# uber-research/UPSNet

Measured on NVIDIA H100. Metric: panoptic images/sec at 1024x2048, higher is better.
Workload: dtype bf16x3

## Files before the change

upsnet_b200/csrc/dcn_win.cu:

```cuda
#include <cuda.h>
#include <cuda_bf16.h>

#include "common.cuh"
#include "tc_ptx.cuh"
#include "tc_params.cuh"

namespace ups {

constexpr int DW_BM = 128;
constexpr int DW_WW = 32, DW_WH = 20;
constexpr int DW_PLANE = DW_WW * DW_WH * 32;
constexpr int DW_WIN_BYTES = 2 * DW_PLANE;
constexpr int DW_WIN_BUFS = 2;
constexpr int DW_KHW = 9;
constexpr int DW_GROUPS = 2;
constexpr int DW_EPI_PITCH = 36;
constexpr uint32_t DW_EPI_BYTES = DW_BM * DW_EPI_PITCH * 4;

constexpr uint32_t DW_OFF_BARS = 0;
constexpr uint32_t DW_OFF_STATS = 192;
constexpr uint32_t DW_OFF_ORG = 256;
constexpr uint32_t DW_OFF_TW = 512;
constexpr uint32_t DW_OFF_TP = DW_OFF_TW + DW_KHW * DW_BM * 16;
constexpr uint32_t DW_OFF_STAGES = DW_OFF_TP + DW_KHW * DW_BM * 4;
static_assert(DW_OFF_STAGES % 1024 == 0, "stage buffers need 1024-byte alignment (SWIZZLE_128B)");

template <int BN> struct DwCfg {
  static constexpr int NCW = BN == 128 ? 2 : 1;
  static constexpr int FRAGS = 2 / NCW;
  static constexpr int BK = BN == 128 ? 32 : 64;
  static constexpr int SPK = BK / 16;
  static constexpr int ROWB = BK * 2;
  static constexpr int CONSUMERS = 128 * NCW;
  static constexpr int WARP_TMAB = CONSUMERS / 32, WARP_TMAW = WARP_TMAB + 1, WARP_PROD0 = WARP_TMAB + 4;
  static constexpr int GROUP = 4 * (SPK / 2) * 32;
  static constexpr int PRODUCERS = GROUP * DW_GROUPS;
  static constexpr int THREADS = WARP_PROD0 * 32 + PRODUCERS;
  static constexpr int WARPGROUPS = THREADS / 128;
  static constexpr int REGS_LAUNCH = 16384 / (32 * ((THREADS / 32 + 3) / 4)) / 8 * 8;
  static constexpr int REGS_TMA = 32, REGS_CONSUMER = 128;
  static_assert(NCW * REGS_CONSUMER + REGS_TMA + (PRODUCERS / 128) * REGS_LAUNCH <= WARPGROUPS * REGS_LAUNCH,
                "setmaxnreg budgets exceed the CTA's register allocation");
  static constexpr int TABLE_IT = (DW_KHW * DW_BM + PRODUCERS - 1) / PRODUCERS;
  static constexpr uint32_t A_BYTES = 2 * DW_BM * ROWB;
  static constexpr uint32_t B_BYTES = BN * ROWB;
  static constexpr uint32_t STAGE_BYTES = 2 * B_BYTES + A_BYTES;
  static_assert(STAGE_BYTES % 1024 == 0, "stages must keep the 1024-byte alignment of the swizzled tiles");
  static constexpr int STAGES = BN == 128 ? 3 : 2;
  static_assert(STAGES <= 3, "the barrier map holds three stages");
  static constexpr uint32_t OFF_WIN = DW_OFF_STAGES + STAGES * STAGE_BYTES;
  static constexpr uint32_t OFF_EPI = OFF_WIN + DW_WIN_BUFS * DW_WIN_BYTES;
  static constexpr uint32_t SMEM = OFF_EPI + DW_EPI_BYTES + 1024;
  static_assert(SMEM <= 227 * 1024, "shared memory exceeds 227 KB");
};
template <int ROWB> __device__ __forceinline__ uint32_t dw_chunk(uint32_t j, uint32_t r) {
  return ROWB == 128 ? (j ^ (r & 7u)) : (j ^ ((r >> 1) & 3u));
}

struct DwParams {
  const void* x;
  const float* offset;
  const float* mask;
  const float* bias;
  void* y;
  int N, H, W, Cin, Cout, Cout_pad, Ho, Wo, ph, pw, dh, dw, relu, BN, tile_w, tile_h;
};

template <int BN>
__global__ void __launch_bounds__(DwCfg<BN>::THREADS, 1)
dcn_win_kernel(const __grid_constant__ CUtensorMap tm_x, const __grid_constant__ CUtensorMap tm_w, const __grid_constant__ DwParams p) {
  using C = DwCfg<BN>;
  constexpr int DW_PRODUCERS = C::PRODUCERS, DW_CONSUMERS = C::CONSUMERS;
  constexpr int DW_WARP_TMAB = C::WARP_TMAB, DW_WARP_TMAW = C::WARP_TMAW, DW_WARP_PROD0 = C::WARP_PROD0;
  constexpr int DW_BK = C::BK, SPK = C::SPK, ROWB = C::ROWB;
  extern __shared__ __align__(1024) uint8_t smem_dyn[];
  const uint32_t raw = smem_u32(smem_dyn);
  const uint32_t base = (raw + 1023u) & ~1023u;
  uint8_t* sm = smem_dyn + (base - raw);

  const int tid = threadIdx.x, warp = tid >> 5, lane = tid & 31;
  const uint32_t b_bytes = C::B_BYTES;
  const uint32_t stage_bytes = C::STAGE_BYTES;
  constexpr uint32_t NST = C::STAGES, NWB = DW_WIN_BUFS;
  const uint32_t win_base = base + C::OFF_WIN;
  float* stf = reinterpret_cast<float*>(sm + C::OFF_EPI);
  const uint32_t bar_fa = base + DW_OFF_BARS;
  const uint32_t bar_fb = bar_fa + 24;
  const uint32_t bar_em = bar_fa + 48;
  const uint32_t bar_wf = bar_fa + 104;
  const uint32_t bar_we = bar_fa + 120;
  const uint32_t bar_og = bar_fa + 136;
  int* stats = reinterpret_cast<int*>(sm + DW_OFF_STATS);
  int4* org = reinterpret_cast<int4*>(sm + DW_OFF_ORG);
  float4* tw = reinterpret_cast<float4*>(sm + DW_OFF_TW);
  int* tp = reinterpret_cast<int*>(sm + DW_OFF_TP);

  const int HoWo = p.Ho * p.Wo;
  const int nsc = p.Cin / 16;
  const int num_kb = nsc * DW_KHW / SPK;
  const int n_tiles = p.Cout_pad / BN;
  const int TW = p.tile_w, TH = p.tile_h;
  const int tw_shift = TW == 16 ? 4 : 3;
  const int tiles_w = (p.Wo + TW - 1) / TW, tiles_h = (p.Ho + TH - 1) / TH;
  const long long num_tiles = (long long)p.N * tiles_w * tiles_h * n_tiles;

  if (warp == 0) {
    if (lane == 0) {
      for (int s = 0; s < C::STAGES; ++s) {
        mbar_init(bar_fa + 8 * s, C::GROUP / 32);
        mbar_init(bar_fb + 8 * s, 1);
        mbar_init(bar_em + 8 * s, DW_CONSUMERS / 32);
      }
      for (int s = 0; s < 2; ++s) {
        mbar_init(bar_wf + 8 * s, 1);
        mbar_init(bar_we + 8 * s, DW_PRODUCERS / 32);
        mbar_init(bar_og + 8 * s, 1);
      }
      fence_mbar_init();
      for (int i = 0; i < 2; ++i) {
        stats[i * 8 + 0] = 0x7fffffff; stats[i * 8 + 1] = 0x7fffffff;
        stats[i * 8 + 2] = -0x7fffffff; stats[i * 8 + 3] = -0x7fffffff;
        stats[i * 8 + 4] = 0; stats[i * 8 + 5] = 0; stats[i * 8 + 6] = 0; stats[i * 8 + 7] = 0;
      }
    }
    __syncwarp();
  }
  if (warp == DW_WARP_TMAB && lane == 0) prefetch_tmap(&tm_w);
  if (warp == DW_WARP_TMAW && lane == 0) prefetch_tmap(&tm_x);
  __syncthreads();

  if (warp >= DW_WARP_PROD0) {
    const int pt = tid - DW_WARP_PROD0 * 32;
    const int pw = warp - DW_WARP_PROD0;
    const int group = pw / (C::GROUP / 32);
    const int u = (pw >> 2) & (SPK / 2 - 1);
    const int quad = pw & 3;
    const int r = quad * 32 + lane;
    const __nv_bfloat16* xh = reinterpret_cast<const __nv_bfloat16*>(p.x);
    uint32_t g0 = 0, wf0 = 0;
    uint32_t wf_ready = 0;
    uint32_t tile_it = 0;
    for (long long tile = blockIdx.x; tile < num_tiles; tile += gridDim.x, ++tile_it) {
      const long long mt = tile / n_tiles;
      const int tx = (int)(mt % tiles_w), ty = (int)((mt / tiles_w) % tiles_h), n = (int)(mt / ((long long)tiles_w * tiles_h));
      const int par = (int)(tile_it & 1u);
      constexpr int TIT = C::TABLE_IT;
      float4 ewv[TIT];
      int ehl[TIT], ewl[TIT];
      bool evalid[TIT];
      int mnw = 0x7fffffff, mnh = 0x7fffffff, mxw = -0x7fffffff, mxh = -0x7fffffff, sw_ = 0, sh_ = 0, cnt = 0;
#pragma unroll
      for (int it = 0; it < TIT; ++it) {
        const int e = pt + it * DW_PRODUCERS;
        ewv[it] = make_float4(0.f, 0.f, 0.f, 0.f);
        ehl[it] = 0; ewl[it] = 0; evalid[it] = false;
        if (e < DW_KHW * DW_BM) {
          const int tap = e >> 7, rr = e & 127;
          const int ry = rr >> tw_shift;
          const int wo = tx * TW + (rr & (TW - 1)), ho = ty * TH + ry;
          if (ry < TH && wo < p.Wo && ho < p.Ho) {
            const int pp = ho * p.Wo + wo;
            const int ki = tap / 3, kj = tap - ki * 3;
            const float* offp = p.offset + ((size_t)n * 2 * DW_KHW + 2 * tap) * HoWo + pp;
            const float oh = __ldg(offp), ow = __ldg(offp + HoWo);
            const float h = (float)(ho - p.ph + ki * p.dh) + oh;
            const float w = (float)(wo - p.pw + kj * p.dw) + ow;
            if (h > -1.f && w > -1.f && h < (float)p.H && w < (float)p.W) {
              const int hl = (int)floorf(h), wl = (int)floorf(w), hh = hl + 1, wh = wl + 1;
              const float lh = h - hl, lw = w - wl, ch = 1.f - lh, cw = 1.f - lw;
              const bool t_ok = hl >= 0, b_ok = hh <= p.H - 1, l_ok = wl >= 0, r_ok = wh <= p.W - 1;
              float m = 1.f;
              if (p.mask) m = __ldg(p.mask + ((size_t)n * DW_KHW + tap) * HoWo + pp);
              ewv[it].x = (t_ok && l_ok) ? ch * cw * m : 0.f;
              ewv[it].y = (t_ok && r_ok) ? ch * lw * m : 0.f;
              ewv[it].z = (b_ok && l_ok) ? lh * cw * m : 0.f;
              ewv[it].w = (b_ok && r_ok) ? lh * lw * m : 0.f;
              ehl[it] = hl; ewl[it] = wl; evalid[it] = true;
              mnw = min(mnw, wl); mxw = max(mxw, wl + 1); mnh = min(mnh, hl); mxh = max(mxh, hl + 1);
              sw_ += wl; sh_ += hl; ++cnt;
            }
          }
        }
      }
      mnw = __reduce_min_sync(0xffffffffu, mnw); mnh = __reduce_min_sync(0xffffffffu, mnh);
      mxw = __reduce_max_sync(0xffffffffu, mxw); mxh = __reduce_max_sync(0xffffffffu, mxh);
      sw_ = __reduce_add_sync(0xffffffffu, sw_); sh_ = __reduce_add_sync(0xffffffffu, sh_);
      cnt = __reduce_add_sync(0xffffffffu, cnt);
      if (lane == 0 && cnt > 0) {
        int* st = stats + par * 8;
        atomicMin(st + 0, mnw); atomicMin(st + 1, mnh); atomicMax(st + 2, mxw); atomicMax(st + 3, mxh);
        atomicAdd(st + 4, sw_); atomicAdd(st + 5, sh_); atomicAdd(st + 6, cnt);
      }
      named_bar<1, DW_PRODUCERS>();
      int ox = 0, oy = 0;
      {
        const int* st = stats + par * 8;
        const int c = st[6];
        if (c > 0) {
          const int a = st[0], b = st[1], cc = st[2], d = st[3];
          ox = (cc - a + 1 <= DW_WW) ? a : (int)floorf((float)st[4] / (float)c + 1.0f) - DW_WW / 2;
          oy = (d - b + 1 <= DW_WH) ? b : (int)floorf((float)st[5] / (float)c + 1.0f) - DW_WH / 2;
        }
      }
#pragma unroll
      for (int it = 0; it < TIT; ++it) {
        const int e = pt + it * DW_PRODUCERS;
        if (e < DW_KHW * DW_BM) {
          int code = 0;
          if (evalid[it]) {
            const int dx = ewl[it] - ox, dy = ehl[it] - oy;
            if (dx >= 0 && dx + 1 < DW_WW && dy >= 0 && dy + 1 < DW_WH) code = (dy * DW_WW + dx) * 32;
            else code = (int)(0x80000000u | ((uint32_t)(ehl[it] + 1) << 15) | (uint32_t)(ewl[it] + 1));
          }
          tw[e] = ewv[it];
          tp[e] = code;
        }
      }
      if (pt == 0) {
        org[par] = make_int4(ox, oy, n, 0);
        int* so = stats + (par ^ 1) * 8;
        so[0] = 0x7fffffff; so[1] = 0x7fffffff; so[2] = -0x7fffffff; so[3] = -0x7fffffff; so[4] = 0; so[5] = 0; so[6] = 0;
        mbar_arrive(bar_og + 8 * par);
      }
      named_bar<1, DW_PRODUCERS>();
      const __nv_bfloat16* ximg = xh + (size_t)n * p.H * p.W * (size_t)(2 * p.Cin);

      int rel = 0;
      for (int kb = (int)((uint32_t)(group - (int)g0) & 1u); kb < num_kb; kb += DW_GROUPS) {
        const uint32_t g = g0 + (uint32_t)kb;
        const uint32_t s = g % NST, it = g / NST;
        mbar_wait(bar_em + 8 * s, (it & 1u) ^ 1u);
        const uint32_t a_row = base + DW_OFF_STAGES + s * stage_bytes + 2 * b_bytes + (uint32_t)r * (uint32_t)ROWB;
#pragma unroll 1
        for (int pass = 0; pass < 4; ++pass) {
          const int sl = 2 * u + (pass >> 1), half = pass & 1;
          const int q = kb * SPK + sl;
          const int sc = q / DW_KHW, tap = q - sc * DW_KHW;
          const uint32_t wf = wf0 + (uint32_t)sc;
          if (wf >= wf_ready) {
            mbar_wait(bar_wf + 8 * (wf % NWB), (wf / NWB) & 1u);
            wf_ready = wf + 1;
          }
          const uint32_t wbuf = win_base + (wf % NWB) * (uint32_t)DW_WIN_BYTES;
          const int code = tp[tap * DW_BM + r];
          const uint32_t a_off = dw_chunk<ROWB>((uint32_t)(sl * 2 + half), (uint32_t)r) << 4;
          const float4 wv = tw[tap * DW_BM + r];
          uint4 hc[4], lc[4];
          if (code >= 0) {
            const uint32_t cl = (uint32_t)code, cr = cl + 32u;
            const uint32_t al = wbuf + cl + ((((cl >> 7) & 1u) ^ (uint32_t)half) << 4);
            const uint32_t ar = wbuf + cr + ((((cr >> 7) & 1u) ^ (uint32_t)half) << 4);
            hc[0] = lds128(al); hc[1] = lds128(ar); hc[2] = lds128(al + DW_WW * 32); hc[3] = lds128(ar + DW_WW * 32);
            lc[0] = lds128(al + DW_PLANE); lc[1] = lds128(ar + DW_PLANE);
            lc[2] = lds128(al + DW_PLANE + DW_WW * 32); lc[3] = lds128(ar + DW_PLANE + DW_WW * 32);
          } else {
            const int hl = (int)(((uint32_t)code >> 15) & 0xffffu) - 1, wl = (int)((uint32_t)code & 0x7fffu) - 1;
            const int h0 = max(hl, 0), h1 = min(hl + 1, p.H - 1), w0 = max(wl, 0), w1 = min(wl + 1, p.W - 1);
            const size_t pc = (size_t)(2 * p.Cin);
            const int cg = sc * 16 + half * 8;
            const __nv_bfloat16* b00 = ximg + ((size_t)h0 * p.W + w0) * pc + cg;
            const __nv_bfloat16* b01 = ximg + ((size_t)h0 * p.W + w1) * pc + cg;
            const __nv_bfloat16* b10 = ximg + ((size_t)h1 * p.W + w0) * pc + cg;
            const __nv_bfloat16* b11 = ximg + ((size_t)h1 * p.W + w1) * pc + cg;
            hc[0] = __ldg(reinterpret_cast<const uint4*>(b00)); lc[0] = __ldg(reinterpret_cast<const uint4*>(b00 + p.Cin));
            hc[1] = __ldg(reinterpret_cast<const uint4*>(b01)); lc[1] = __ldg(reinterpret_cast<const uint4*>(b01 + p.Cin));
            hc[2] = __ldg(reinterpret_cast<const uint4*>(b10)); lc[2] = __ldg(reinterpret_cast<const uint4*>(b10 + p.Cin));
            hc[3] = __ldg(reinterpret_cast<const uint4*>(b11)); lc[3] = __ldg(reinterpret_cast<const uint4*>(b11 + p.Cin));
          }
          const float wf4[4] = {wv.x, wv.y, wv.z, wv.w};
          unsigned long long acc[4] = {0ull, 0ull, 0ull, 0ull};
          __nv_bfloat162 lacc[4];
#pragma unroll
          for (int i = 0; i < 4; ++i) {
            const uint32_t hw_[4] = {hc[i].x, hc[i].y, hc[i].z, hc[i].w};
            const uint32_t lw_[4] = {lc[i].x, lc[i].y, lc[i].z, lc[i].w};
            const __nv_bfloat162 wb = __float2bfloat162_rn(wf4[i]);
            unsigned long long wp;
            asm("mov.b64 %0, {%1, %1};" : "=l"(wp) : "r"(__float_as_uint(wf4[i])));
#pragma unroll
            for (int qq = 0; qq < 4; ++qq) {
              unsigned long long hp;
              asm("mov.b64 %0, {%1, %2};" : "=l"(hp) : "r"(hw_[qq] << 16), "r"(hw_[qq] & 0xffff0000u));
              acc[qq] = f32x2_fma(wp, hp, acc[qq]);
              const __nv_bfloat162 lv = *reinterpret_cast<const __nv_bfloat162*>(&lw_[qq]);
              lacc[qq] = i == 0 ? __hmul2(wb, lv) : __hfma2(wb, lv, lacc[qq]);
            }
          }
          uint32_t ohi[4], olo[4];
#pragma unroll
          for (int qq = 0; qq < 4; ++qq) {
            const uint32_t lw = *reinterpret_cast<const uint32_t*>(&lacc[qq]);
            unsigned long long lp;
            asm("mov.b64 %0, {%1, %2};" : "=l"(lp) : "r"(lw << 16), "r"(lw & 0xffff0000u));
            acc[qq] = f32x2_add(acc[qq], lp);
            uint32_t a0, a1;
            asm("mov.b64 {%0, %1}, %2;" : "=r"(a0), "=r"(a1) : "l"(acc[qq]));
            const float v0 = __uint_as_float(a0), v1 = __uint_as_float(a1);
            ohi[qq] = pack_bf16x2(v0, v1);
            olo[qq] = pack_bf16x2(v0 - __uint_as_float(ohi[qq] << 16), v1 - __uint_as_float(ohi[qq] & 0xffff0000u));
          }
          sts128(a_row + a_off, make_uint4(ohi[0], ohi[1], ohi[2], ohi[3]));
          sts128(a_row + DW_BM * ROWB + a_off, make_uint4(olo[0], olo[1], olo[2], olo[3]));
        }
        fence_proxy_async();
        __syncwarp();
        if (lane == 0) {
          mbar_arrive(bar_fa + 8 * s);
          while (rel < nsc && DW_KHW * (rel + 1) <= SPK * (kb + DW_GROUPS)) {
            mbar_arrive(bar_we + 8 * ((wf0 + (uint32_t)rel) % NWB));
            ++rel;
          }
        }
        rel = __shfl_sync(0xffffffffu, rel, 0);
      }
      if (lane == 0) {
        while (rel < nsc) { mbar_arrive(bar_we + 8 * ((wf0 + (uint32_t)rel) % NWB)); ++rel; }
      }
      __syncwarp();
      g0 += (uint32_t)num_kb;
      wf0 += (uint32_t)nsc;
    }
  } else if (warp >= DW_WARP_TMAB) {
    setmaxnreg_dec<C::REGS_TMA>();
    if (warp == DW_WARP_TMAW && lane == 0) {
      uint32_t wf = 0, ti = 0;
      for (long long tile = blockIdx.x; tile < num_tiles; tile += gridDim.x, ++ti) {
        const uint32_t par = ti & 1u;
        mbar_wait(bar_og + 8 * par, (ti >> 1) & 1u);
        const volatile int* ov = reinterpret_cast<const volatile int*>(&org[par]);
        const int4 o = make_int4(ov[0], ov[1], ov[2], 0);
        for (int f = 0; f < nsc; ++f, ++wf) {
          const uint32_t b = wf % NWB;
          mbar_wait(bar_we + 8 * b, ((wf / NWB) & 1u) ^ 1u);
          mbar_arrive_expect_tx(bar_wf + 8 * b, (uint32_t)DW_WIN_BYTES);
          const uint32_t dst = win_base + b * (uint32_t)DW_WIN_BYTES;
          tma_load_4d(dst, &tm_x, bar_wf + 8 * b, f * 16, o.x, o.y, o.z);
          tma_load_4d(dst + (uint32_t)DW_PLANE, &tm_x, bar_wf + 8 * b, p.Cin + f * 16, o.x, o.y, o.z);
        }
      }
    } else if (warp == DW_WARP_TMAB && lane == 0) {
      uint32_t g = 0;
      for (long long tile = blockIdx.x; tile < num_tiles; tile += gridDim.x) {
        const int n0 = (int)(tile % n_tiles) * BN;
        for (int kb = 0; kb < num_kb; ++kb, ++g) {
          const uint32_t s = g % NST, it = g / NST;
          mbar_wait(bar_em + 8 * s, (it & 1u) ^ 1u);
          const uint32_t stage = base + DW_OFF_STAGES + s * stage_bytes;
          mbar_arrive_expect_tx(bar_fb + 8 * s, 2 * b_bytes);
          tma_load_2d(stage, &tm_w, bar_fb + 8 * s, kb * DW_BK, n0);
          tma_load_2d(stage + b_bytes, &tm_w, bar_fb + 8 * s, kb * DW_BK, p.Cout_pad + n0);
        }
      }
    }
    __syncwarp();
  } else {
    setmaxnreg_inc<C::REGS_CONSUMER>();
    constexpr int FRAGS = C::FRAGS;
    const int wg = warp >> 2;
    const uint32_t dhi = ROWB == 128 ? wg_desc_hi(8 * ROWB) : wg_desc_hi_sw64(8 * ROWB);
    float d[FRAGS][BN / 2];
    constexpr uint32_t h16 = 64u * ROWB / 16u;
    __nv_bfloat16* yb = reinterpret_cast<__nv_bfloat16*>(p.y);
    uint32_t s = 0, ph = 0;
    for (long long tile = blockIdx.x; tile < num_tiles; tile += gridDim.x) {
      const long long mt = tile / n_tiles;
      const int n0 = (int)(tile % n_tiles) * BN;
      const int tx = (int)(mt % tiles_w), ty = (int)((mt / tiles_w) % tiles_h), n = (int)(mt / ((long long)tiles_w * tiles_h));
      int prev = -1;
      for (int kb = 0; kb < num_kb; ++kb) {
        mbar_wait(bar_fb + 8 * s, ph);
        mbar_wait(bar_fa + 8 * s, ph);
        const uint32_t st0 = base + DW_OFF_STAGES + s * stage_bytes;
        const uint32_t b_hi = wg_desc_lo(st0), b_lo = wg_desc_lo(st0 + b_bytes);
        const uint32_t a_hi = wg_desc_lo(st0 + 2 * b_bytes) + (uint32_t)(wg * FRAGS) * h16;
        const uint32_t a_lo = wg_desc_lo(st0 + 2 * b_bytes + DW_BM * ROWB) + (uint32_t)(wg * FRAGS) * h16;
        wgmma_fence();
#pragma unroll
        for (uint32_t k = 0; k < SPK; ++k) {
          const uint32_t acc = (kb | k) ? 1u : 0u;
          const uint64_t bh = wg_desc(b_hi + 2 * k, dhi), bl = wg_desc(b_lo + 2 * k, dhi);
#pragma unroll
          for (int f = 0; f < FRAGS; ++f) Wgmma<BN>::mma(d[f], wg_desc(a_lo + f * h16 + 2 * k, dhi), bh, acc);
#pragma unroll
          for (int f = 0; f < FRAGS; ++f) Wgmma<BN>::mma(d[f], wg_desc(a_hi + f * h16 + 2 * k, dhi), bl, 1u);
#pragma unroll
          for (int f = 0; f < FRAGS; ++f) Wgmma<BN>::mma(d[f], wg_desc(a_hi + f * h16 + 2 * k, dhi), bh, 1u);
        }
        wgmma_commit();
        wgmma_wait<1>();
#pragma unroll
        for (int f = 0; f < FRAGS; ++f) wgmma_fence_acc(d[f]);
        if (prev >= 0 && lane == 0) mbar_arrive(bar_em + 8 * prev);
        prev = (int)s;
        if (++s == NST) { s = 0; ph ^= 1u; }
      }
      wgmma_wait<0>();
#pragma unroll
      for (int f = 0; f < FRAGS; ++f) wgmma_fence_acc(d[f]);
      if (prev >= 0 && lane == 0) mbar_arrive(bar_em + 8 * prev);

      const int t = tid & 127;
      const int m = FRAGS == 2 ? t : 64 * wg + (t & 63);
      const int csub = FRAGS == 2 ? 0 : 16 * (t >> 6), cstep = FRAGS == 2 ? 16 : 32;
      const int ry = m >> tw_shift;
      const int wo = tx * TW + (m & (TW - 1)), ho = ty * TH + ry;
      const bool row_ok = ry < TH && wo < p.Wo && ho < p.Ho;
      __nv_bfloat16* yp = yb + (((size_t)n * p.Ho + ho) * p.Wo + wo) * (size_t)(2 * p.Cout);
      const uint32_t trow = smem_u32(stf + (size_t)m * DW_EPI_PITCH);
      for (int c32 = 0; c32 < BN; c32 += 32) {
        if (n0 + c32 >= p.Cout) break;
        named_bar(2 + wg, 128);
#pragma unroll
        for (int c = 0; c < BN; c += 32)
          if (c == c32) {
#pragma unroll
            for (int f = 0; f < FRAGS; ++f) acc_stage<BN, 32>(d[f], stf, DW_EPI_PITCH, 64 * (wg * FRAGS + f), c);
          }
        named_bar(2 + wg, 128);
        for (int cb = c32 + csub; cb < c32 + 32 && cb < BN; cb += cstep) {
          if (n0 + cb >= p.Cout) break;
          uint32_t rr[16];
          acc_ld16(trow + (uint32_t)(cb - c32) * 4u, rr);
          if (!row_ok) continue;
          const int co = n0 + cb;
          float o[16];
#pragma unroll
          for (int e = 0; e < 16; ++e) o[e] = __uint_as_float(rr[e]);
          if (p.bias) {
            if (co + 16 <= p.Cout) {
#pragma unroll
              for (int e4 = 0; e4 < 4; ++e4) {
                const float4 bv = __ldg(reinterpret_cast<const float4*>(p.bias + co) + e4);
                o[4 * e4] += bv.x; o[4 * e4 + 1] += bv.y; o[4 * e4 + 2] += bv.z; o[4 * e4 + 3] += bv.w;
              }
            } else {
#pragma unroll
              for (int e = 0; e < 16; ++e)
                if (co + e < p.Cout) o[e] += __ldg(p.bias + co + e);
            }
          }
          if (p.relu) {
#pragma unroll
            for (int e = 0; e < 16; ++e) o[e] = fmaxf(o[e], 0.f);
          }
          uint32_t hw[8], lw[8];
#pragma unroll
          for (int e = 0; e < 8; ++e) {
            hw[e] = pack_bf16x2(o[2 * e], o[2 * e + 1]);
            lw[e] = pack_bf16x2(o[2 * e] - __uint_as_float(hw[e] << 16), o[2 * e + 1] - __uint_as_float(hw[e] & 0xffff0000u));
          }
          uint4* dh_ = reinterpret_cast<uint4*>(yp + co);
          uint4* dl_ = reinterpret_cast<uint4*>(yp + p.Cout + co);
          dh_[0] = make_uint4(hw[0], hw[1], hw[2], hw[3]); dh_[1] = make_uint4(hw[4], hw[5], hw[6], hw[7]);
          dl_[0] = make_uint4(lw[0], lw[1], lw[2], lw[3]); dl_[1] = make_uint4(lw[4], lw[5], lw[6], lw[7]);
        }
      }
    }
  }
}

__global__ void dcn_win_pack_kernel(const float* __restrict__ w, int Cout, int Cin, int Cout_pad, int K,
                                    uint16_t* __restrict__ hi, uint16_t* __restrict__ lo) {
  const size_t total = (size_t)Cout_pad * K;
  for (size_t i = (size_t)blockIdx.x * blockDim.x + threadIdx.x; i < total; i += (size_t)gridDim.x * blockDim.x) {
    const int kk = (int)(i % (size_t)K), co = (int)(i / (size_t)K);
    const int sc = kk / (16 * DW_KHW), rem = kk - sc * 16 * DW_KHW, tap = rem >> 4, c = sc * 16 + (rem & 15);
    const float v = co < Cout ? w[((size_t)co * Cin + c) * DW_KHW + tap] : 0.f;
    const __nv_bfloat16 h = __float2bfloat16_rn(v);
    const __nv_bfloat16 l = __float2bfloat16_rn(v - __bfloat162float(h));
    hi[i] = *reinterpret_cast<const uint16_t*>(&h);
    lo[i] = *reinterpret_cast<const uint16_t*>(&l);
  }
}

static bool dw_supported(int Cin, int Cout, int kh, int kw) {
  return kh == 3 && kw == 3 && Cin % 64 == 0 && Cin >= 64 && Cout >= 1;
}

}

extern "C" int upsnet_dcn_packed_weight_bytes(int Cout, int Cin, int kh, int kw, size_t* bytes) {
  if (!bytes || Cout <= 0 || Cin <= 0) return UPSNET_E_BADARG;
  if (!ups::dw_supported(Cin, Cout, kh, kw)) return UPSNET_E_UNSUPPORTED;
  *bytes = (size_t)2 * ups::cout_pad(Cout) * (size_t)(9 * Cin) * sizeof(uint16_t);
  return 0;
}

extern "C" int upsnet_dcn_pack_weight(const float* weight, int Cout, int Cin, int kh, int kw, void* packed, void* stream) {
  if (!weight || !packed || Cout <= 0 || Cin <= 0) return UPSNET_E_BADARG;
  if (!ups::dw_supported(Cin, Cout, kh, kw)) return UPSNET_E_UNSUPPORTED;
  const int Cout_pad = ups::cout_pad(Cout), K = 9 * Cin;
  uint16_t* hi = reinterpret_cast<uint16_t*>(packed);
  uint16_t* lo = hi + (size_t)Cout_pad * K;
  const size_t total = (size_t)Cout_pad * K;
  int blocks = (int)((total + 255) / 256);
  if (blocks > ups::kNumSMs * 16) blocks = ups::kNumSMs * 16;
  ups::dcn_win_pack_kernel<<<blocks, 256, 0, (cudaStream_t)stream>>>(weight, Cout, Cin, Cout_pad, K, hi, lo);
  UPS_CHECK_LAUNCH();
  return 0;
}

static int g_dw_force_bn = 0;

extern "C" int upsnet_dcn_set_tile_n(int bn) {
  if (bn != 0 && bn != 32 && bn != 128) return UPSNET_E_BADARG;
  g_dw_force_bn = bn;
  return 0;
}

extern "C" int upsnet_dcn_pair_forward(const void* x_pair, const float* offset, const float* mask, const void* packed,
                                       const float* bias, void* y_pair, int N, int H, int W, int Cin, int Cout, int kh,
                                       int kw, int pad_h, int pad_w, int dil_h, int dil_w, int epi_flags, void* stream) {
  using namespace ups;
  if (!x_pair || !offset || !packed || !y_pair) return UPSNET_E_BADARG;
  if (N <= 0 || H <= 0 || W <= 0 || Cin <= 0 || Cout <= 0 || pad_h < 0 || pad_w < 0 || dil_h <= 0 || dil_w <= 0) return UPSNET_E_BADARG;
  if (!dw_supported(Cin, Cout, kh, kw)) return UPSNET_E_UNSUPPORTED;
  if ((Cout % 16) != 0) return UPSNET_E_UNSUPPORTED;
  if (H >= 32767 || W >= 32767) return UPSNET_E_UNSUPPORTED;
  if ((((uintptr_t)x_pair) & 15) || (((uintptr_t)packed) & 15) || (((uintptr_t)y_pair) & 15) || (bias && (((uintptr_t)bias) & 15)))
    return UPSNET_E_UNSUPPORTED;
  DwParams p{};
  p.x = x_pair; p.offset = offset; p.mask = mask; p.bias = bias; p.y = y_pair;
  p.N = N; p.H = H; p.W = W; p.Cin = Cin; p.Cout = Cout; p.Cout_pad = cout_pad(Cout);
  p.ph = pad_h; p.pw = pad_w; p.dh = dil_h; p.dw = dil_w;
  p.Ho = conv_out_size(H, pad_h, dil_h, 3, 1);
  p.Wo = conv_out_size(W, pad_w, dil_w, 3, 1);
  if (p.Ho <= 0 || p.Wo <= 0) return UPSNET_E_BADARG;
  p.relu = (epi_flags & UPSNET_EPI_RELU) ? 1 : 0;
  const int sms = num_sms();
  p.tile_w = 16; p.tile_h = 8;
  auto dtiles = [&]() { return (long long)p.N * ((p.Wo + p.tile_w - 1) / p.tile_w) * ((p.Ho + p.tile_h - 1) / p.tile_h) * (p.Cout_pad / p.BN); };
  p.BN = 128;
  const bool wide_ok = p.Cout_pad % 128 == 0;
  const bool wide = wide_ok && (g_dw_force_bn == 128 || (g_dw_force_bn == 0 && dtiles() >= sms / 4));
  if (!wide) p.BN = 32;
  if (!wide && dtiles() < sms / 2) { p.tile_w = 8; p.tile_h = 8; }
  if (!wide && dtiles() < sms / 2) { p.tile_h = 4; }
  const long long num_tiles = dtiles();
  if (num_tiles <= 0) return 0;
  const int bk = wide ? DwCfg<128>::BK : DwCfg<32>::BK;
  const size_t smem = wide ? DwCfg<128>::SMEM : DwCfg<32>::SMEM;
  EncodeTiledFn enc = tma_encoder();
  if (!enc) return UPSNET_E_UNSUPPORTED;
  CUtensorMap tm_x, tm_w;
  {
    const cuuint64_t dx[4] = {(cuuint64_t)(2 * Cin), (cuuint64_t)W, (cuuint64_t)H, (cuuint64_t)N};
    const cuuint64_t sx[3] = {(cuuint64_t)(2 * Cin) * 2, (cuuint64_t)W * (2 * Cin) * 2, (cuuint64_t)H * W * (2 * Cin) * 2};
    const cuuint32_t bx[4] = {16, DW_WW, DW_WH, 1};
    const cuuint32_t es[4] = {1, 1, 1, 1};
    if (enc(&tm_x, CU_TENSOR_MAP_DATA_TYPE_BFLOAT16, 4, const_cast<void*>(x_pair), dx, sx, bx, es, CU_TENSOR_MAP_INTERLEAVE_NONE,
            CU_TENSOR_MAP_SWIZZLE_32B, CU_TENSOR_MAP_L2_PROMOTION_L2_128B, CU_TENSOR_MAP_FLOAT_OOB_FILL_NONE) != CUDA_SUCCESS)
      return UPSNET_E_UNSUPPORTED;
    const cuuint64_t dwt[2] = {(cuuint64_t)(9 * Cin), (cuuint64_t)(2 * p.Cout_pad)};
    const cuuint64_t sw[1] = {(cuuint64_t)(9 * Cin) * 2};
    const cuuint32_t bw[2] = {(cuuint32_t)bk, (cuuint32_t)p.BN};
    if (enc(&tm_w, CU_TENSOR_MAP_DATA_TYPE_BFLOAT16, 2, const_cast<void*>(packed), dwt, sw, bw, es, CU_TENSOR_MAP_INTERLEAVE_NONE,
            bk == 64 ? CU_TENSOR_MAP_SWIZZLE_128B : CU_TENSOR_MAP_SWIZZLE_64B, CU_TENSOR_MAP_L2_PROMOTION_L2_256B,
            CU_TENSOR_MAP_FLOAT_OOB_FILL_NONE) != CUDA_SUCCESS)
      return UPSNET_E_UNSUPPORTED;
  }
  static PerDeviceOnce configured;
  if (configured.need()) {
    UPS_CUDA(cudaFuncSetAttribute(dcn_win_kernel<32>, cudaFuncAttributeMaxDynamicSharedMemorySize, 227 * 1024));
    UPS_CUDA(cudaFuncSetAttribute(dcn_win_kernel<128>, cudaFuncAttributeMaxDynamicSharedMemorySize, 227 * 1024));
  }
  dim3 grid((unsigned)(num_tiles < sms ? num_tiles : sms));
  if (wide)
    dcn_win_kernel<128><<<grid, DwCfg<128>::THREADS, smem, (cudaStream_t)stream>>>(tm_x, tm_w, p);
  else
    dcn_win_kernel<32><<<grid, DwCfg<32>::THREADS, smem, (cudaStream_t)stream>>>(tm_x, tm_w, p);
  UPS_CHECK_LAUNCH();
  return 0;
}
```

Measured before the change: 127.9.

## Software-pipeline DCN producer window loads across passes and k-blocks

Restructures the deformable-conv producer loop so the high-plane corner loads for the next pass (and the next k-block when its window is already resident) are issued before the low-plane bf16 accumulation of the current pass. The pass loop is fully unrolled and the slice lookup is factored into lambdas. This is meant to hide shared-memory load latency behind FMA work. It also packs the per-entry hl/wl/valid into a single int and replaces a divide by 3 with a multiply-shift, at the cost of more live registers and more complex carry logic.

```diff
diff --git a/upsnet_b200/csrc/dcn_win.cu b/upsnet_b200/csrc/dcn_win.cu
--- a/upsnet_b200/csrc/dcn_win.cu
+++ b/upsnet_b200/csrc/dcn_win.cu
@@ -146,21 +146,21 @@
       const int par = (int)(tile_it & 1u);
       constexpr int TIT = C::TABLE_IT;
       float4 ewv[TIT];
-      int ehl[TIT], ewl[TIT];
-      bool evalid[TIT];
+      int ehw[TIT];
+
       int mnw = 0x7fffffff, mnh = 0x7fffffff, mxw = -0x7fffffff, mxh = -0x7fffffff, sw_ = 0, sh_ = 0, cnt = 0;
 #pragma unroll
       for (int it = 0; it < TIT; ++it) {
         const int e = pt + it * DW_PRODUCERS;
         ewv[it] = make_float4(0.f, 0.f, 0.f, 0.f);
-        ehl[it] = 0; ewl[it] = 0; evalid[it] = false;
+        ehw[it] = -1;
         if (e < DW_KHW * DW_BM) {
           const int tap = e >> 7, rr = e & 127;
           const int ry = rr >> tw_shift;
           const int wo = tx * TW + (rr & (TW - 1)), ho = ty * TH + ry;
           if (ry < TH && wo < p.Wo && ho < p.Ho) {
             const int pp = ho * p.Wo + wo;
-            const int ki = tap / 3, kj = tap - ki * 3;
+            const int ki = (tap * 11) >> 5, kj = tap - ki * 3;
             const float* offp = p.offset + ((size_t)n * 2 * DW_KHW + 2 * tap) * HoWo + pp;
             const float oh = __ldg(offp), ow = __ldg(offp + HoWo);
             const float h = (float)(ho - p.ph + ki * p.dh) + oh;
@@ -175,7 +175,7 @@
               ewv[it].y = (t_ok && r_ok) ? ch * lw * m : 0.f;
               ewv[it].z = (b_ok && l_ok) ? lh * cw * m : 0.f;
               ewv[it].w = (b_ok && r_ok) ? lh * lw * m : 0.f;
-              ehl[it] = hl; ewl[it] = wl; evalid[it] = true;
+              ehw[it] = ((hl + 1) << 16) | (wl + 1);
               mnw = min(mnw, wl); mxw = max(mxw, wl + 1); mnh = min(mnh, hl); mxh = max(mxh, hl + 1);
               sw_ += wl; sh_ += hl; ++cnt;
             }
@@ -207,10 +207,11 @@
         const int e = pt + it * DW_PRODUCERS;
         if (e < DW_KHW * DW_BM) {
           int code = 0;
-          if (evalid[it]) {
-            const int dx = ewl[it] - ox, dy = ehl[it] - oy;
+          if (ehw[it] >= 0) {
+            const int hl = (ehw[it] >> 16) - 1, wl = (ehw[it] & 0xffff) - 1;
+            const int dx = wl - ox, dy = hl - oy;
             if (dx >= 0 && dx + 1 < DW_WW && dy >= 0 && dy + 1 < DW_WH) code = (dy * DW_WW + dx) * 32;
-            else code = (int)(0x80000000u | ((uint32_t)(ehl[it] + 1) << 15) | (uint32_t)(ewl[it] + 1));
+            else code = (int)(0x80000000u | ((uint32_t)(hl + 1) << 15) | (uint32_t)(wl + 1));
           }
           tw[e] = ewv[it];
           tp[e] = code;
@@ -225,56 +226,76 @@
       named_bar<1, DW_PRODUCERS>();
       const __nv_bfloat16* ximg = xh + (size_t)n * p.H * p.W * (size_t)(2 * p.Cin);
 
+      auto win_corners = [&](int code, int half, uint32_t wbuf, uint32_t plane, uint4 (&c)[4]) {
+        const uint32_t cl = (uint32_t)code, cr = cl + 32u;
+        const uint32_t al = wbuf + plane + cl + ((((cl >> 7) & 1u) ^ (uint32_t)half) << 4);
+        const uint32_t ar = wbuf + plane + cr + ((((cr >> 7) & 1u) ^ (uint32_t)half) << 4);
+        c[0] = lds128(al); c[1] = lds128(ar); c[2] = lds128(al + DW_WW * 32); c[3] = lds128(ar + DW_WW * 32);
+      };
+      auto global_corners = [&](int code, int half, int sc, uint4 (&hc_)[4], uint4 (&lc_)[4]) {
+        const int hl = (int)(((uint32_t)code >> 15) & 0xffffu) - 1, wl = (int)((uint32_t)code & 0x7fffu) - 1;
+        const int h0 = max(hl, 0), h1 = min(hl + 1, p.H - 1), w0 = max(wl, 0), w1 = min(wl + 1, p.W - 1);
+        const size_t pc = (size_t)(2 * p.Cin);
+        const int cg = sc * 16 + half * 8;
+        const __nv_bfloat16* b00 = ximg + ((size_t)h0 * p.W + w0) * pc + cg;
+        const __nv_bfloat16* b01 = ximg + ((size_t)h0 * p.W + w1) * pc + cg;
+        const __nv_bfloat16* b10 = ximg + ((size_t)h1 * p.W + w0) * pc + cg;
+        const __nv_bfloat16* b11 = ximg + ((size_t)h1 * p.W + w1) * pc + cg;
+        hc_[0] = __ldg(reinterpret_cast<const uint4*>(b00)); lc_[0] = __ldg(reinterpret_cast<const uint4*>(b00 + p.Cin));
+        hc_[1] = __ldg(reinterpret_cast<const uint4*>(b01)); lc_[1] = __ldg(reinterpret_cast<const uint4*>(b01 + p.Cin));
+        hc_[2] = __ldg(reinterpret_cast<const uint4*>(b10)); lc_[2] = __ldg(reinterpret_cast<const uint4*>(b10 + p.Cin));
+        hc_[3] = __ldg(reinterpret_cast<const uint4*>(b11)); lc_[3] = __ldg(reinterpret_cast<const uint4*>(b11 + p.Cin));
+      };
+      auto slice = [&](int kb_, int sl_, int& sc_, int& tap_, int& code_, uint32_t& wbuf_) {
+        const int q = kb_ * SPK + sl_;
+        sc_ = q / DW_KHW;
+        tap_ = q - sc_ * DW_KHW;
+        code_ = tp[tap_ * DW_BM + r];
+        const uint32_t wf = wf0 + (uint32_t)sc_;
+        if (wf >= wf_ready) {
+          mbar_wait(bar_wf + 8 * (wf % NWB), (wf / NWB) & 1u);
+          wf_ready = wf + 1;
+        }
+        wbuf_ = win_base + (wf % NWB) * (uint32_t)DW_WIN_BYTES;
+      };
+
       int rel = 0;
-      for (int kb = (int)((uint32_t)(group - (int)g0) & 1u); kb < num_kb; kb += DW_GROUPS) {
+      const int kb0 = (int)((uint32_t)(group - (int)g0) & 1u);
+      int sc = 0, tap = 0, code = 0;
+      float4 wv = make_float4(0.f, 0.f, 0.f, 0.f);
+      uint32_t wbuf = 0;
+      uint4 hc[4];
+      bool carried = false;
+      for (int kb = kb0; kb < num_kb; kb += DW_GROUPS) {
+        if (!carried) {
+          slice(kb, 2 * u, sc, tap, code, wbuf);
+          wv = tw[tap * DW_BM + r];
+          if (code >= 0) win_corners(code, 0, wbuf, 0u, hc);
+        }
         const uint32_t g = g0 + (uint32_t)kb;
         const uint32_t s = g % NST, it = g / NST;
         mbar_wait(bar_em + 8 * s, (it & 1u) ^ 1u);
         const uint32_t a_row = base + DW_OFF_STAGES + s * stage_bytes + 2 * b_bytes + (uint32_t)r * (uint32_t)ROWB;
-#pragma unroll 1
+#pragma unroll
         for (int pass = 0; pass < 4; ++pass) {
           const int sl = 2 * u + (pass >> 1), half = pass & 1;
-          const int q = kb * SPK + sl;
-          const int sc = q / DW_KHW, tap = q - sc * DW_KHW;
-          const uint32_t wf = wf0 + (uint32_t)sc;
-          if (wf >= wf_ready) {
-            mbar_wait(bar_wf + 8 * (wf % NWB), (wf / NWB) & 1u);
-            wf_ready = wf + 1;
-          }
-          const uint32_t wbuf = win_base + (wf % NWB) * (uint32_t)DW_WIN_BYTES;
-          const int code = tp[tap * DW_BM + r];
-          const uint32_t a_off = dw_chunk<ROWB>((uint32_t)(sl * 2 + half), (uint32_t)r) << 4;
-          const float4 wv = tw[tap * DW_BM + r];
-          uint4 hc[4], lc[4];
-          if (code >= 0) {
-            const uint32_t cl = (uint32_t)code, cr = cl + 32u;
-            const uint32_t al = wbuf + cl + ((((cl >> 7) & 1u) ^ (uint32_t)half) << 4);
-            const uint32_t ar = wbuf + cr + ((((cr >> 7) & 1u) ^ (uint32_t)half) << 4);
-            hc[0] = lds128(al); hc[1] = lds128(ar); hc[2] = lds128(al + DW_WW * 32); hc[3] = lds128(ar + DW_WW * 32);
-            lc[0] = lds128(al + DW_PLANE); lc[1] = lds128(ar + DW_PLANE);
-            lc[2] = lds128(al + DW_PLANE + DW_WW * 32); lc[3] = lds128(ar + DW_PLANE + DW_WW * 32);
-          } else {
-            const int hl = (int)(((uint32_t)code >> 15) & 0xffffu) - 1, wl = (int)((uint32_t)code & 0x7fffu) - 1;
-            const int h0 = max(hl, 0), h1 = min(hl + 1, p.H - 1), w0 = max(wl, 0), w1 = min(wl + 1, p.W - 1);
-            const size_t pc = (size_t)(2 * p.Cin);
-            const int cg = sc * 16 + half * 8;
-            const __nv_bfloat16* b00 = ximg + ((size_t)h0 * p.W + w0) * pc + cg;
-            const __nv_bfloat16* b01 = ximg + ((size_t)h0 * p.W + w1) * pc + cg;
-            const __nv_bfloat16* b10 = ximg + ((size_t)h1 * p.W + w0) * pc + cg;
-            const __nv_bfloat16* b11 = ximg + ((size_t)h1 * p.W + w1) * pc + cg;
-            hc[0] = __ldg(reinterpret_cast<const uint4*>(b00)); lc[0] = __ldg(reinterpret_cast<const uint4*>(b00 + p.Cin));
-            hc[1] = __ldg(reinterpret_cast<const uint4*>(b01)); lc[1] = __ldg(reinterpret_cast<const uint4*>(b01 + p.Cin));
-            hc[2] = __ldg(reinterpret_cast<const uint4*>(b10)); lc[2] = __ldg(reinterpret_cast<const uint4*>(b10 + p.Cin));
-            hc[3] = __ldg(reinterpret_cast<const uint4*>(b11)); lc[3] = __ldg(reinterpret_cast<const uint4*>(b11 + p.Cin));
-          }
+          uint4 lc[4];
+          if (code >= 0) win_corners(code, half, wbuf, (uint32_t)DW_PLANE, lc);
+          else global_corners(code, half, sc, hc, lc);
+          int sc1 = sc, tap1 = tap, code1 = code;
+          uint32_t wbuf1 = wbuf;
+          if (pass == 3) {
+            const int f1 = ((kb + DW_GROUPS) * SPK + 2 * u) / DW_KHW;
+            carried = kb + DW_GROUPS < num_kb && DW_KHW * (f1 - 1) <= SPK * kb;
+          }
+          const bool more = pass < 3 || carried;
+          if (pass == 1) slice(kb, sl + 1, sc1, tap1, code1, wbuf1);
+          else if (pass == 3 && more) slice(kb + DW_GROUPS, 2 * u, sc1, tap1, code1, wbuf1);
           const float wf4[4] = {wv.x, wv.y, wv.z, wv.w};
           unsigned long long acc[4] = {0ull, 0ull, 0ull, 0ull};
-          __nv_bfloat162 lacc[4];
 #pragma unroll
           for (int i = 0; i < 4; ++i) {
             const uint32_t hw_[4] = {hc[i].x, hc[i].y, hc[i].z, hc[i].w};
-            const uint32_t lw_[4] = {lc[i].x, lc[i].y, lc[i].z, lc[i].w};
-            const __nv_bfloat162 wb = __float2bfloat162_rn(wf4[i]);
             unsigned long long wp;
             asm("mov.b64 %0, {%1, %1};" : "=l"(wp) : "r"(__float_as_uint(wf4[i])));
 #pragma unroll
@@ -282,6 +303,18 @@
               unsigned long long hp;
               asm("mov.b64 %0, {%1, %2};" : "=l"(hp) : "r"(hw_[qq] << 16), "r"(hw_[qq] & 0xffff0000u));
               acc[qq] = f32x2_fma(wp, hp, acc[qq]);
+            }
+          }
+          asm volatile("" : "+l"(acc[0]), "+l"(acc[1]), "+l"(acc[2]), "+l"(acc[3]));
+          if (more && code1 >= 0) win_corners(code1, half ^ 1, wbuf1, 0u, hc);
+          const float4 wv1 = (pass & 1) && more ? tw[tap1 * DW_BM + r] : wv;
+          __nv_bfloat162 lacc[4];
+#pragma unroll
+          for (int i = 0; i < 4; ++i) {
+            const uint32_t lw_[4] = {lc[i].x, lc[i].y, lc[i].z, lc[i].w};
+            const __nv_bfloat162 wb = __float2bfloat162_rn(wf4[i]);
+#pragma unroll
+            for (int qq = 0; qq < 4; ++qq) {
               const __nv_bfloat162 lv = *reinterpret_cast<const __nv_bfloat162*>(&lw_[qq]);
               lacc[qq] = i == 0 ? __hmul2(wb, lv) : __hfma2(wb, lv, lacc[qq]);
             }
@@ -299,8 +332,10 @@
             ohi[qq] = pack_bf16x2(v0, v1);
             olo[qq] = pack_bf16x2(v0 - __uint_as_float(ohi[qq] << 16), v1 - __uint_as_float(ohi[qq] & 0xffff0000u));
           }
+          const uint32_t a_off = dw_chunk<ROWB>((uint32_t)(sl * 2 + half), (uint32_t)r) << 4;
           sts128(a_row + a_off, make_uint4(ohi[0], ohi[1], ohi[2], ohi[3]));
           sts128(a_row + DW_BM * ROWB + a_off, make_uint4(olo[0], olo[1], olo[2], olo[3]));
+          sc = sc1; tap = tap1; code = code1; wv = wv1; wbuf = wbuf1;
         }
         fence_proxy_async();
         __syncwarp();
```

After: 129.0 (median of 6 runs). About the same (+0.9%).
